# eduard-permyakov/permafrost-engine

Hardware: AMD Instinct MI355X
Metric: agent-steps/sec (+ flow-field cells/sec), every chunk field rebuilt + every agent stepped per tick (higher is better)
Workload: dtype u64-bitmask/u8 fields, f32 agents (f64 exp); 1 GPU; BASELINE configs[2]: 1024x1024 cells, 64 flow fields = 16384 chunk fields, 100000 agents; map_chunks=16, flow_fields=64, agents=100000, hz=20, dynamic_obstacles=0, parallelism=requests by destination + uid slabs x1, 1 all-gather (16 B/agent) per tick, ranks=1, rccl_ranks=1, backend=none, tile_exchange=auto, requests=reference planner fixture, has_dest_los=device lookup, initial_velocities=flow aligned, fields_ahead=True, tick_driver=c (navhip_tick_run), library=libnavhip.so (in-tree)

## Files before the change

permafrost-engine_amd/csrc/agent_internal.h:

```cpp
#pragma once
#define NH_SCAN_T 256
#include "navhip_internal.h"
#include "agent_types.h"

struct nh_spatial_scratch {
    int32_t *ent_cell, *ent_rank;
    int32_t *cell_count;
    int32_t *cell_start;
    int32_t *tmp_id;
    int32_t *block_sum;
    int32_t *box;
    int      box_parity;
    float4  *recA;
    float2  *recV;
    int32_t *pool_of;
    nh_pack_src src;
};

void nh_launch_spatial_build(nh_grid &G, const float *d_pos_xz, nh_spatial_scratch &S,
                             int slab_begin, int slab_end, hipStream_t s);
void nh_launch_agent_nbr(const nh_step_params &P, const nh_nbr &NB, hipStream_t s);
size_t nh_cohesion_scratch_bytes(int n_flocks, int n_members);
hipError_t nh_cohesion_scratch_reset(int32_t *scratch, int n_flocks, int n_members, hipStream_t s);
bool nh_launch_cohesion(const nh_step_params &P, int32_t *scratch, float *d_coh, int *parity, hipStream_t s);
void nh_launch_cohesion_regroup(const nh_step_params &P, int32_t *scratch, int *parity, hipStream_t s);
int nh_worklist_cap(int n_work);
bool nh_launch_agent_finish(const nh_step_params &P, const nh_nbr &NB, float *d_coh, nh_mid_rec *d_mid,
                            nh_worklists WL, int parity, const nh_step_outs &O, hipStream_t s,
                            hipStream_t side, navhip_ctx *ctx, bool *forked);
void nh_launch_state_update(const nh_step_params &P, const navhip_state_in &in, float4 *d_arrived, int32_t *d_arrived_n, uint8_t *d_state, uint8_t *d_flags,
                            hipStream_t s);
void nh_launch_region_lookup(const nh_step_params &P, int nq, const float *d_pos, const int32_t *d_rows,
                             const int32_t *d_centre_abs, const int32_t *d_radius, uint8_t *d_dir, uint8_t *d_at_slot,
                             hipStream_t s);
void nh_launch_spatial_query(const nh_grid &G, const float *d_query, int nq, float range, int maxout,
                             int32_t *d_counts, uint32_t *d_ids, hipStream_t s);
void nh_launch_clearpath(int nq, const float *ent, const float *des_v, const float *dyn,
                         const int32_t *n_dyn, const float *stat, const int32_t *n_stat, float *out,
                         int rows, hipStream_t s);
```

permafrost-engine_amd/csrc/agent_kernels.hip:

```cpp
#include "navhip_internal.h"
#include "agent_internal.h"
#include "agent_group.h"

__constant__ double c_exp2_64[64] = { NH_EXP2_64_TABLE };

#define SP_MAX_QUERY_R 30
__global__ __launch_bounds__(256) void k_sp_bbox(const float *pos_xz, int begin, int end, int32_t *box)
{
    __shared__ int32_t part[4][4];
    int32_t v[4] = {INT32_MIN, INT32_MIN, INT32_MIN, INT32_MIN};
    for(int i = begin + blockIdx.x * 256 + threadIdx.x; i < end; i += gridDim.x * 256) {
        const int32_t ix = bg_scale(pos_xz[2 * i]), iy = bg_scale(pos_xz[2 * i + 1]);
        v[0] = max(v[0], -ix); v[1] = max(v[1], ix); v[2] = max(v[2], -iy); v[3] = max(v[3], iy);
    }
#pragma unroll
    for(int q = 0; q < 4; q++) {
#pragma unroll
        for(int d = 32; d >= 1; d >>= 1) v[q] = max(v[q], __shfl_xor(v[q], d));
        if((threadIdx.x & 63) == 0) part[threadIdx.x >> 6][q] = v[q];
    }
    __syncthreads();
    if(threadIdx.x < 4) {
        int32_t m = INT32_MIN;
        for(int w = 0; w < 4; w++) m = max(m, part[w][threadIdx.x]);
// ... 900 lines not shown
    unit_totals(unit_end, 2 * NH_WL_SUB, [&](int k) { return (sub_cnt[k] + 3) >> 2; });
    __syncthreads();
    const int u = blockIdx.x * CPS_WAVES + wib;
    bool live = u < unit_end[2 * NH_WL_SUB - 1];
    int uid = 0;
    bool found = true;
    if(live) {
        const int k = first_above(unit_end, 2 * NH_WL_SUB, u), rel = u - (k ? unit_end[k - 1] : 0);
        const int list = NH_WL_ROW1 - k / NH_WL_SUB, sub = k % NH_WL_SUB;
        const int idx = rel * 4 + (lane >> 4);
        live = idx < sub_cnt[k];
        if(live) {
            uid = WL.ids[((size_t)list * NH_WL_SUB + sub) * WL.cap + idx];
            const nh_mid_rec R = mid[uid];
            const uint32_t c = NB.cnt[uid];
            const int n_dyn = (int)(c & 0xff), n_stat = (int)((c >> 8) & 0xff);
            cpent ent;
            ent.pos = mkv(P.pos_xz[2 * uid], P.pos_xz[2 * uid + 1]);
            ent.vel = mkv(P.vel_xz[2 * uid], P.vel_xz[2 * uid + 1]);
            ent.radius = P.radius[uid];
            const int gl = lane & 15;
            const bool have = gl < n_dyn + n_stat, isdyn = gl < n_dyn;
            cpent nb; nb.pos = mkv(0, 0); nb.vel = mkv(0, 0); nb.radius = 0;
            if(have) nb = nbr_load(NB, uid, isdyn ? gl : 32 + gl - n_dyn);
            const v2 nv = clearpath_small_row(ent, mkv(R.vpref[0], R.vpref[1]), nb, isdyn, have,
                                              cones[wib * 4 + (lane >> 4)], found);
            if(found && gl == 0)
                post_thread(P, uid, ent.pos, P.state[uid], P.flags[uid], ent.radius, nv, R.vel_cap, R.status, O);
        }
    }
    worklist_push(WL, NH_WL_RETRY, live && !found && (lane & 15) == 0, uid);
}

#define CP_ROWS_OCC 4
__attribute__((amdgpu_waves_per_eu(CP_ROWS_OCC, CP_ROWS_OCC)))
__global__ __launch_bounds__(CPR_WAVES * 64) void k_cp_rows(nh_step_params P, nh_nbr NB, const nh_mid_rec *mid,
                                                           nh_worklists WL, nh_step_outs O, int list0, int nlists,
                                                           int ticket_set, nh_signal lists_ready)
{
    if(lists_ready.flag && blockIdx.x == 0 && threadIdx.x == 0) {
#ifdef NH_HOSTSIM
        *lists_ready.flag = lists_ready.seq;
#else
        __hip_atomic_store(lists_ready.flag, lists_ready.seq, __ATOMIC_RELEASE, __HIP_MEMORY_SCOPE_AGENT);
#endif
    }
    __shared__ cp_lds<16> lds[CPR_WAVES * 4];
    __shared__ int32_t unit_end[4 * NH_WL_SUB];
    __shared__ int32_t sub_cnt[4 * NH_WL_SUB];
    asm volatile("" ::: "v127");
    static_assert(sizeof(cp_lds<16>) * CPR_WAVES * 4 + 8 * 4 * NH_WL_SUB >= sizeof(cp_lds<64>) * CP_WAVES + 8 * NH_WL_SUB + 4 + sizeof(cp_team),
                  "k_cp_rows' workgroup must own at least k_cp_heavy's LDS (hole inheritance)");
    const int wib = threadIdx.x >> 6, lane = threadIdx.x & 63;
    const int ntab = nlists * NH_WL_SUB;
    if(nlists == 1 && !__any(WL.count[list0 * NH_WL_SUB + lane] != 0)) return;
    for(int k = threadIdx.x; k < ntab; k += CPR_WAVES * 64)
        sub_cnt[k] = WL.count[(list0 - k / NH_WL_SUB) * NH_WL_SUB + k % NH_WL_SUB];
    __syncthreads();
    unit_totals(unit_end, ntab, [&](int k) { return (sub_cnt[k] + 3) >> 2; });
    __syncthreads();
    const int total = unit_end[ntab - 1];
    int32_t *counters = WL.count + NH_WL_LISTS * NH_WL_SUB + 32 * (1 + ticket_set * NH_CP_STRIPES);
    const int gw = blockIdx.x * CPR_WAVES + wib, nw = gridDim.x * CPR_WAVES;
    cp_lds<16> &S = lds[wib * 4 + (lane >> 4)];
    unit_draw D; D.round = 0;
    for(;;) {
        const int u = next_unit(D, counters, total, gw, nw, lane);
        if(u < 0) break;
        const int k = first_above(unit_end, ntab, u), rel = u - (k ? unit_end[k - 1] : 0);
        const int list = list0 - k / NH_WL_SUB, sub = k % NH_WL_SUB;
        const int idx = rel * 4 + (lane >> 4);
        if(idx < sub_cnt[k]) {
            const int uid = WL.ids[((size_t)list * NH_WL_SUB + sub) * WL.cap + idx];
            const nh_mid_rec R = mid[uid];
            const uint32_t c = NB.cnt[uid];
            const int n_dyn = (int)(c & 0xff), n_stat = (int)((c >> 8) & 0xff);
            cpent ent;
            ent.pos = mkv(P.pos_xz[2 * uid], P.pos_xz[2 * uid + 1]);
            ent.vel = mkv(P.vel_xz[2 * uid], P.vel_xz[2 * uid + 1]);
            ent.radius = P.radius[uid];
            cp_load_lists<16>(P.grid, NB, uid, n_dyn, n_stat, S);
            const v2 nv = clearpath_grp<16>(ent, mkv(R.vpref[0], R.vpref[1]), n_dyn, n_stat, S);
            if((lane & 15) == 0)
                post_thread(P, uid, ent.pos, P.state[uid], P.flags[uid], ent.radius, nv, R.vel_cap, R.status, O);
        }
    }
}

#define CP_HEAVY_OCC 4
__attribute__((amdgpu_waves_per_eu(CP_HEAVY_OCC, CP_HEAVY_OCC)))
__global__ __launch_bounds__(CP_WAVES * 64) void k_cp_heavy(nh_step_params P, nh_nbr NB, const nh_mid_rec *mid,
                                                            nh_worklists WL, nh_step_outs O, int32_t *zero_next)
{
    __shared__ cp_lds<64> lds[CP_WAVES];
    __shared__ int32_t hv_end[2 * NH_WL_SUB];
    __shared__ int32_t h_ticket;
    __shared__ cp_team team;
    const int wib = threadIdx.x >> 6, lane = threadIdx.x & 63;
    if(blockIdx.x == 0 && zero_next)
        for(int i = threadIdx.x; i < (int)NH_WL_COUNTERS; i += CP_WAVES * 64) zero_next[i] = 0;
    cp_lds<64> &S = lds[wib];
    if(!__any((WL.count[NH_WL_HEAVY * NH_WL_SUB + lane] | WL.count[NH_WL_WAVE * NH_WL_SUB + lane]) != 0)) return;
    unit_totals(hv_end, 2 * NH_WL_SUB, [&](int k) {
        return WL.count[(k < NH_WL_SUB ? NH_WL_HEAVY : NH_WL_WAVE) * NH_WL_SUB + k % NH_WL_SUB]; });
    __syncthreads();
    const int n_heavy = hv_end[2 * NH_WL_SUB - 1];
    int32_t *ticket = WL.count + NH_WL_LISTS * NH_WL_SUB;
    if(n_heavy >= CP_SOLO_MIN) {
        const int nw = (int)gridDim.x * CP_WAVES;
        for(int round = 0; ; round++) {
            int t = (int)blockIdx.x * CP_WAVES + wib;
            if(round > 0) {
                int v = 0x7fffffff;
                if(lane == 0 && nw + __atomic_load_n(ticket, __ATOMIC_RELAXED) < n_heavy) v = nw + atomicAdd(ticket, 1);
                t = __shfl(v, 0);
            }
            if(t >= n_heavy) break;
            const int k = first_above(hv_end, 2 * NH_WL_SUB, t), idx = t - (k ? hv_end[k - 1] : 0);
            const int uid = WL.ids[((size_t)(k < NH_WL_SUB ? NH_WL_HEAVY : NH_WL_WAVE) * NH_WL_SUB + k % NH_WL_SUB) * WL.cap + idx];
            const nh_mid_rec R = mid[uid];
            const uint32_t c = NB.cnt[uid];
            const int n_dyn = (int)(c & 0xff), n_stat = (int)((c >> 8) & 0xff);
            cpent ent;
            ent.pos = mkv(P.pos_xz[2 * uid], P.pos_xz[2 * uid + 1]);
            ent.vel = mkv(P.vel_xz[2 * uid], P.vel_xz[2 * uid + 1]);
            ent.radius = P.radius[uid];
            cp_load_lists<64>(P.grid, NB, uid, n_dyn, n_stat, S);
            const v2 nv = clearpath_grp<64>(ent, mkv(R.vpref[0], R.vpref[1]), n_dyn, n_stat, S);
            if(lane == 0)
                post_thread(P, uid, ent.pos, P.state[uid], P.flags[uid], ent.radius, nv, R.vel_cap, R.status, O);
        }
        return;
    }
    for(int round = 0; ; round++) {
        int t = blockIdx.x;
        if(round > 0) {
            __syncthreads();
            if(threadIdx.x == 0) {
                int v = 0x7fffffff;
                if((int)gridDim.x + __atomic_load_n(ticket, __ATOMIC_RELAXED) < n_heavy)
                    v = (int)gridDim.x + atomicAdd(ticket, 1);
                h_ticket = v;
            }
            __syncthreads();
            t = h_ticket;
        }
        if(t >= n_heavy) break;
        const int k = first_above(hv_end, 2 * NH_WL_SUB, t), idx = t - (k ? hv_end[k - 1] : 0);
        const int uid = WL.ids[((size_t)(k < NH_WL_SUB ? NH_WL_HEAVY : NH_WL_WAVE) * NH_WL_SUB + k % NH_WL_SUB) * WL.cap + idx];
        const nh_mid_rec R = mid[uid];
        const uint32_t c = NB.cnt[uid];
        const int n_dyn = (int)(c & 0xff), n_stat = (int)((c >> 8) & 0xff);
        cpent ent;
        ent.pos = mkv(P.pos_xz[2 * uid], P.pos_xz[2 * uid + 1]);
        ent.vel = mkv(P.vel_xz[2 * uid], P.vel_xz[2 * uid + 1]);
        ent.radius = P.radius[uid];
        const v2 vpref = mkv(R.vpref[0], R.vpref[1]);
        cp_load_lists<64>(P.grid, NB, uid, n_dyn, n_stat, S);
        const v2 nv = clearpath_grp<64, true>(ent, vpref, n_dyn, n_stat, S, wib, CP_WAVES, &team);
        if(wib == 0 && lane == 0)
            post_thread(P, uid, ent.pos, P.state[uid], P.flags[uid], ent.radius, nv, R.vel_cap, R.status, O);
    }
}

__global__ __launch_bounds__(AG_WAVES * 64) void k_agent_full(nh_step_params P, const float *coh_xz,
                                                              const nh_mid_rec *mid, nh_worklists WL,
                                                              nh_step_outs O, float scaled_max_force,
                                                              double force_thresh, int32_t *zero_next)
{
    __shared__ wave_lds lds[AG_WAVES];
    __shared__ cp_lds<64> cps[AG_WAVES];
    __shared__ double exp_tab[64];
    const int wib = threadIdx.x >> 6, lane = threadIdx.x & 63;
    if(blockIdx.x == 0 && zero_next)
        for(int i = threadIdx.x; i < (int)NH_WL_COUNTERS; i += AG_WAVES * 64) zero_next[i] = 0;
    if(!__any(WL.count[NH_WL_FULL * NH_WL_SUB + lane] != 0)) return;
    if(threadIdx.x < 64) exp_tab[threadIdx.x] = c_exp2_64[threadIdx.x];
    __syncthreads();
    wave_lds &W = lds[wib];
    cp_lds<64> &S = cps[wib];
    const nh_grid &G = P.grid;
    for(int sub = 0; sub < NH_WL_SUB; sub++) {
    const int count = WL.count[NH_WL_FULL * NH_WL_SUB + sub];
    for(int idx = blockIdx.x * AG_WAVES + wib; idx < count; idx += gridDim.x * AG_WAVES) {
        const int uid = WL.ids[((size_t)NH_WL_FULL * NH_WL_SUB + sub) * WL.cap + idx];
        const nh_mid_rec R = mid[uid];
        const uint32_t my_slot = (uint32_t)G.pool_of[uid];
        const uint32_t my_bits = slot_bits(G, my_slot);
        const v2 me = mkv(P.pos_xz[2 * uid], P.pos_xz[2 * uid + 1]);
        const v2 vel = mkv(P.vel_xz[2 * uid], P.vel_xz[2 * uid + 1]);
        const float my_radius = P.radius[uid];
        int n30raw = -1;
        v2 vpref = mkv(0.0f, 0.0f);
        wave_sync();
        if(R.mode != AM_ZERO_VPREF) {
            int n30 = sp_query_wave(G, me.x, me.z, 30.0f, 128, W.ids30, lane, W.d2_30);
            wave_sync();
            n30raw = n30;
            const int n10d = derive_r10(G, me, W.ids30, W.d2_30, n30raw, W.ids10d, lane);
            n30 = filter_garrisoned_wave(G, W.ids30, n30, lane);
            if(n10d < 0) n30raw = -1; else n30raw = n10d;
            const v2 separation = separation_wave(G, my_slot, me, my_radius, my_bits, W.ids30, n30,
                                                  W.u.sep, scaled_max_force, lane, exp_tab);
            vpref = vpref_from_forces(P, uid, R.mode, me, vel, P.flock[uid], mkv(R.arrive[0], R.arrive[1]),
                                      separation, R.probes, coh_xz, scaled_max_force, force_thresh);
        }
        uint32_t *ids10 = W.u.ids10;
        int n10;
        if(n30raw >= 0) {
            ids10 = W.ids10d;
            n10 = n30raw;
        }else{
            n10 = sp_query_wave(G, me.x, me.z, 10.0f, 512, W.u.ids10, lane);
            wave_sync();
        }
        n10 = filter_garrisoned_wave(G, ids10, n10, lane);
        int n_dyn, n_stat;
        classify_neighbours(G, my_slot, my_bits, ids10, n10, S.dyn, n_dyn, S.stat, n_stat, lane);
        cpent ent; ent.pos = me; ent.vel = vel; ent.radius = my_radius;
        const v2 nv = clearpath_grp<64>(ent, vpref, n_dyn, n_stat, S);
        if(lane == 0) {
            if(O.vpref_xz) { O.vpref_xz[2 * uid] = vpref.x; O.vpref_xz[2 * uid + 1] = vpref.z; }
            post_thread(P, uid, me, P.state[uid], P.flags[uid], my_radius, nv, R.vel_cap, R.status, O);
        }
    }
    }
}

__global__ __launch_bounds__(256) void k_spatial_query(nh_grid G, const float *query_xz, int nq,
                                                       float range, int maxout, int32_t *out_counts,
                                                       uint32_t *out_ids)
{
    const int q = (blockIdx.x * 256 + threadIdx.x) >> 6, lane = threadIdx.x & 63;
    if(q >= nq) return;
    uint32_t *mine = out_ids + (size_t)q * maxout;
    int n = sp_query_wave(G, query_xz[2 * q], query_xz[2 * q + 1], range, maxout, mine, lane);
    wave_sync();
    for(int k = lane; k < n; k += 64) mine[k] = slot_bits(G, mine[k]) >> NH_PB_UID_SHIFT;
    if(lane == 0) out_counts[q] = n;
}

__global__ __launch_bounds__(256) void k_arrived_compact(nh_step_params P, float4 *arrived, int32_t *arrived_n)
{
    __shared__ int count;
    const int f = blockIdx.x;
    if(threadIdx.x == 0) count = 0;
    __syncthreads();
    const int b = P.flock_offsets[f], e = P.flock_offsets[f + 1];
    for(int k0 = b; k0 < e; k0 += 256) {
        const int k = k0 + (int)threadIdx.x;
        int m = -1;
        if(k < e) { m = P.flock_members[k]; if(P.state[m] != NAVHIP_STATE_ARRIVED) m = -1; }
        const uint64_t bal = __ballot(m >= 0);
        int base = 0;
        if((threadIdx.x & 63) == 0 && bal) base = atomicAdd(&count, __popcll(bal));
        base = __shfl(base, 0);
        if(m >= 0) {
            const int at = b + base + __popcll(bal & ((1ull << (threadIdx.x & 63)) - 1ull));
            if(at < P.n_ents) arrived[at] = make_float4(P.pos_xz[2 * m], P.pos_xz[2 * m + 1], P.radius[m], __int_as_float(m));
// ... 298 lines not shown
{
    if(!(P.n_ents > 0 && P.n_flocks > 0 && P.n_members > 0)) return false;
    const coh_scratch C = coh_layout(scratch, P.n_flocks, P.n_members);
    const int nwaves = (P.n_members + 15) / 16 + P.n_flocks;
    const int prev = *parity ^ 1;
    if(P.n_flocks <= COH_INLINE_PLAN_MAX) {
        hipLaunchKernelGGL(k_cohesion<true>, dim3(nwaves), dim3(64), 0, s, P, (const int32_t*)C.wave_off,
                           (const int32_t*)C.perm[prev], (const int32_t*)C.valid, d_coh, (const int32_t*)C.bin_start,
                           (const int32_t*)C.saved[prev]);
        return true;
    }
    hipLaunchKernelGGL(k_coh_plan, dim3(1), dim3(256), 0, s, (const int32_t*)C.bin_start, P.flock_offsets,
                       (const int32_t*)C.saved[prev], P.n_flocks, P.work_begin, P.work_end, P.members_key, C.wave_off, C.valid);
    hipLaunchKernelGGL(k_cohesion<false>, dim3(nwaves), dim3(64), 0, s, P, (const int32_t*)C.wave_off,
                       (const int32_t*)C.perm[prev], (const int32_t*)C.valid, d_coh, (const int32_t*)C.bin_start,
                       (const int32_t*)C.saved[prev]);
    return true;
}

void nh_launch_cohesion_regroup(const nh_step_params &P, int32_t *scratch, int *parity, hipStream_t s)
{
    const coh_scratch C = coh_layout(scratch, P.n_flocks, P.n_members);
    coh_regroup(P, C, *parity, s);
    *parity ^= 1;
}
int nh_worklist_cap(int n_work)
{
    const int waves = (n_work + 63) / 64;
    return ((waves + NH_WL_SUB - 1) / NH_WL_SUB) * 64 + 16;
}

bool nh_launch_agent_finish(const nh_step_params &P, const nh_nbr &NB, float *d_coh, nh_mid_rec *d_mid,
                            nh_worklists WL, int parity, const nh_step_outs &O, hipStream_t s,
                            hipStream_t side, navhip_ctx *ctx, bool *forked)
{
    const int nwork = P.work_end - P.work_begin;
    if(!(P.n_ents > 0 && nwork > 0)) return false;
    const float smf = (float)((double)(0.75f / (float)P.hz) * 20.0);
    const double thresh = ((double)(0.75f / (float)P.hz) * 20.0) * 0.01;
    int32_t *zero_next = WL.count + (parity ^ 1) * NH_WL_COUNTERS;
    WL.count += parity * NH_WL_COUNTERS;
    hipLaunchKernelGGL(k_agent_mid, dim3((nwork + 63) / 64), dim3(64), 0, s, P, NB, (const float*)d_coh, d_mid, WL, O, smf, thresh);
    const bool fork = side != nullptr && side != s;
    hipStream_t sh = fork ? side : s;
    const nh_signal lists_ready = fork ? nh_handover_by_kernel(ctx, NH_HO_MID, s) : nh_signal{nullptr, 0};
    *forked = fork;
    const int nblk = min(4096 / CP_WAVES, (nwork + 15) / 16 + 1);
    const int nblk_rows = min(4096 / CPR_WAVES, (nwork + 15) / 16 * (CP_WAVES / CPR_WAVES) + 1);
    hipLaunchKernelGGL(k_cp_rows, dim3(nblk_rows), dim3(CPR_WAVES * 64), 0, s, P, NB, (const nh_mid_rec*)d_mid, WL, O,
                       (int)NH_WL_ROW3, 2, 0, lists_ready);
    if(fork) nh_handover_wait(ctx, NH_HO_MID, sh);
    hipLaunchKernelGGL(k_cp_small, dim3((nwork / 4 + 2 * NH_WL_SUB + CPS_WAVES - 1) / CPS_WAVES + 1), dim3(CPS_WAVES * 64), 0, sh, P, NB,
                       (const nh_mid_rec*)d_mid, WL, O);
    hipLaunchKernelGGL(k_cp_rows, dim3(64 * CP_WAVES / CPR_WAVES), dim3(CPR_WAVES * 64), 0, sh, P, NB, (const nh_mid_rec*)d_mid, WL, O,
                       (int)NH_WL_RETRY, 1, 1, nh_signal{nullptr, 0});
    hipLaunchKernelGGL(k_cp_heavy, dim3(nblk), dim3(CP_WAVES * 64), 0, sh, P, NB, (const nh_mid_rec*)d_mid, WL, O, zero_next);
    if(fork) nh_handover_signal(ctx, NH_HO_CP, sh);
    hipLaunchKernelGGL(k_agent_full, dim3(min(1024, (nwork + AG_WAVES - 1) / AG_WAVES)), dim3(AG_WAVES * 64), 0, s, P,
                       (const float*)d_coh, (const nh_mid_rec*)d_mid, WL, O, smf, thresh, (int32_t*)nullptr);
    if(fork) nh_handover_wait(ctx, NH_HO_CP, s, -1, NH_HO_END);
    return true;
}

void nh_launch_spatial_query(const nh_grid &G, const float *d_query, int nq, float range, int maxout,
                             int32_t *d_counts, uint32_t *d_ids, hipStream_t s)
{
    if(nq > 0)
        hipLaunchKernelGGL(k_spatial_query, dim3((nq + 3) / 4), dim3(256), 0, s, G, d_query, nq, range,
                           maxout, d_counts, d_ids);
}

void nh_launch_clearpath(int nq, const float *ent, const float *des_v, const float *dyn,
                         const int32_t *n_dyn, const float *stat, const int32_t *n_stat, float *out,
                         int rows, hipStream_t s)
{
    if(nq <= 0) return;
    if(rows == 2)
        hipLaunchKernelGGL(k_clearpath_team, dim3(nq), dim3(CP_WAVES * 64), 0, s, nq, ent, des_v, dyn,
                           n_dyn, stat, n_stat, out);
    else if(rows)
        hipLaunchKernelGGL(k_clearpath<16>, dim3((nq + 7) / 8), dim3(128), 0, s, nq, ent, des_v, dyn,
                           n_dyn, stat, n_stat, out);
    else
        hipLaunchKernelGGL(k_clearpath<64>, dim3((nq + 1) / 2), dim3(128), 0, s, nq, ent, des_v, dyn,
                           n_dyn, stat, n_stat, out);
}
```

permafrost-engine_amd/csrc/agent_types.h:

```cpp
#pragma once
#include <stdint.h>
#include <stddef.h>
#include "map_view.h"

#ifdef NH_HOSTSIM
struct float2 { float x, y; };
struct float4 { float x, y, z, w; };
static inline float2 make_float2(float x, float y) { float2 r = {x, y}; return r; }
static inline float4 make_float4(float x, float y, float z, float w) { float4 r = {x, y, z, w}; return r; }
#endif

#define NH_PB_MOVABLE     0x01u
#define NH_PB_AIR         0x02u
#define NH_PB_GARRISONED  0x04u
#define NH_PB_STATIC      0x08u
#define NH_PB_WATER       0x10u
#define NH_PB_IDLE        0x20u
#define NH_PB_UID_SHIFT   8

struct nh_grid {
    int32_t origin_x, origin_y;
    int     grid_w, grid_h;
    int     n;
    const int32_t *cell_start;
// ... 36 lines not shown
    const float    *los_pos_xz;
    const int32_t  *region_row;
    const int32_t  *region_field_slot;
};

struct nh_step_outs {
    float   *vel_xz, *new_pos_xz, *vdes_xz, *vpref_xz;
    uint8_t *status;
};

#define NH_NB_IRREGULAR 0x1u
#define NH_NB_DONE      0x2u
struct nh_nbr {
    float2   *sep;
    uint32_t *cnt;
    float    *rec;
    int       stride;
};

enum { NH_WL_ROW0 = 0, NH_WL_ROW1, NH_WL_ROW2, NH_WL_ROW3,
       NH_WL_WAVE,
       NH_WL_HEAVY,
       NH_WL_FULL,
       NH_WL_RETRY,
       NH_WL_LISTS };
#define NH_WL_SUB 64
struct nh_worklists {
    int32_t *count;
    int32_t *ids;
    int      cap;
};
#define NH_CP_STRIPES 32
#define NH_WL_COUNTERS (NH_WL_LISTS * NH_WL_SUB + 32 * (2 + 2 * NH_CP_STRIPES))

struct nh_mid_rec {
    float    vpref[2];
    float    vdes[2];
    float    arrive[2];
    uint16_t probes;
    uint8_t  status;
    uint8_t  mode;
    float    vel_cap;
};
```

permafrost-engine_amd/csrc/navhip_internal.h:

```cpp
#pragma once
#include <hip/hip_runtime.h>
#include <stdint.h>
#include <string>
#include <vector>
#include <initializer_list>
#include <stddef.h>
#include "navhip.h"
#include "map_view.h"

static_assert(sizeof(navhip_field_req) == 32, "navhip_field_req must stay 32 bytes");
static_assert(sizeof(navhip_los_req) == 16, "navhip_los_req must stay 16 bytes");

#define NH_CELLS   4096
#define NH_RES     64
#define NH_INF_U32 0x3fffffffu

#define HIPCHK(ctx, expr)                                                                   \
    do {                                                                                    \
        hipError_t _e = (expr);                                                             \
        if(_e != hipSuccess) {                                                              \
            (ctx)->last_error = std::string(#expr) + ": " + hipGetErrorString(_e);          \
            return NAVHIP_ERR_DEVICE;                                                       \
        }                                                                                   \
    } while(0)
// ... 200 lines not shown
{
    nh_buf *one[] = {&ctx->d_reqs, &ctx->d_dirs, &ctx->d_integ, &ctx->d_dirty_list, &ctx->gen_list, &ctx->state_arrived,
                     &ctx->state_arrived_n};
    for(nh_buf *b : one) f(*b);
    for(auto &b : ctx->step.buf) f(b);
    for(auto &b : ctx->stage) f(b);
}

enum { NH_STREAM_SIDE0 = 0,
       NH_STREAM_SIDE1,
       NH_STREAM_MAIN,
       NH_STREAM_FIELDS,
       NH_STREAM_COMM,
       NH_STREAM_FIXED };
int         nh_streams_for(navhip_ctx *ctx, hipStream_t main, hipStream_t out[NH_STREAM_FIXED]);
hipStream_t nh_stream_partial_for(navhip_ctx *ctx, hipStream_t main, int cu_begin, int cu_count);
bool        nh_streams_alive(int device);
void        nh_streams_forget(int device, hipStream_t s);
int         nh_ensure_side_streams(navhip_ctx *ctx, hipStream_t main);

struct nh_signal { int32_t *flag; int32_t seq; };
struct nh_handover {
    int32_t *flags;
    int32_t *status;
    int32_t *status_dev;
    int32_t  seq[NH_HO_FLAGS];
    bool       forced_events, never_events, by_events;
    hipEvent_t ev[NH_HO_FLAGS];
};
void     nh_handover_mode(navhip_ctx *ctx, bool jam);
int      nh_handover_ensure(navhip_ctx *ctx);
void     nh_handover_destroy(navhip_ctx *ctx);
nh_signal nh_handover_by_kernel(navhip_ctx *ctx, int flag, hipStream_t producer);
void     nh_handover_signal(navhip_ctx *ctx, int flag, hipStream_t producer);
void     nh_handover_wait(navhip_ctx *ctx, int flag, hipStream_t consumer, int before = -1, int after = -1);
void     nh_handover_wait2(navhip_ctx *ctx, int flag_a, int flag_b, hipStream_t consumer);
int32_t  nh_handover_seq(navhip_ctx *ctx, int flag);
void     nh_handover_wait_for(navhip_ctx *ctx, int flag, int32_t want, hipStream_t consumer);
bool     nh_handover_failed(navhip_ctx *ctx);

extern "C" int nh_validate_field_reqs(navhip_ctx *ctx, const navhip_field_req *reqs, int n);
int  navhip_build_fields_slots_dev(navhip_ctx *ctx, const navhip_field_req *dev_reqs, int n, uint8_t *dev_fields,
                                   const int32_t *dev_slots, hipStream_t s);
int  nh_ensure(navhip_ctx *ctx, nh_buf &b, size_t need);
int  nh_ensure_buf(navhip_ctx *ctx, nh_buf &b, size_t need);
int  nh_stage_in(navhip_ctx *ctx, nh_stage_slot slot, const void *host, size_t bytes, const void **dst, hipStream_t s);
int  nh_stage_world(navhip_ctx *ctx, const navhip_world *w, navhip_world *d, hipStream_t s, std::initializer_list<size_t> only = {});
int  nh_stage_reserve(navhip_ctx *ctx, nh_stage_slot slot, size_t bytes, void **dev);
void nh_async_destroy(navhip_ctx *ctx);
void nh_async_invalidate_static(navhip_ctx *ctx);
bool nh_async_resident(navhip_ctx *ctx, navhip_world *w, navhip_step_out *o);
int  nh_async_slabs(navhip_ctx *ctx, size_t in_bytes, size_t out_bytes, char **h_in, char **h_out);
bool nh_is_pinned(const void *p);
int  nh_refresh_derived(navhip_ctx *ctx, hipStream_t s);
int  nh_spatial_query_dev(navhip_ctx *ctx, const navhip_world *dev_w, const float *d_query, int nq, float range, int maxout,
                          int32_t *d_counts, uint32_t *d_ids, hipStream_t s);
const uint8_t *nh_pool_fields(const navhip_ctx *ctx);
const int32_t *nh_pool_map(const navhip_ctx *ctx);
int nh_pool_dests(const navhip_ctx *ctx);
int nh_pool_slots(const navhip_ctx *ctx);

void nh_launch_derive(navhip_ctx *ctx, int layer, const uint32_t *d_chunk_list, int n,
                      hipStream_t s);
int  nh_launch_fields(navhip_ctx *ctx, const navhip_field_req *d_reqs, int n, uint8_t *d_dirs,
                      float *d_integ, int32_t *d_gen_list, hipStream_t s,
                      const int32_t *d_out_slot = nullptr);

void nh_launch_blockers_circles(navhip_ctx *ctx, const navhip_circle *d_circles, int n, float map_x,
                                float map_z, hipStream_t s);
// ... 8 lines not shown
```

permafrost-engine_amd/csrc/step_api.hip:

```cpp
#include "navhip_internal.h"
#include "agent_internal.h"
#include "agent_thread.h"
#include <cmath>

#include <algorithm>
#include <cstring>
#include <initializer_list>

enum sb_fresh : uint8_t {
    SB_ANYTHING,
    SB_ZEROED,
    SB_EMPTY_BOXES,
};
struct sb_need { nh_step_buf buf; size_t bytes; sb_fresh fresh; };

template<size_t N> static int step_bufs_ensure(navhip_ctx *ctx, const sb_need (&needs)[N], hipStream_t s)
{
    for(const sb_need &n : needs) {
        nh_buf &b = ctx->step.buf[n.buf];
        const void *old = b.p;
        int rc = nh_ensure_buf(ctx, b, n.bytes);
        if(rc) return rc;
        if(b.p == old) continue;
        if(n.fresh == SB_ZEROED) HIPCHK(ctx, hipMemsetAsync(b.p, 0, b.cap, s));
// ... 306 lines not shown
        HIPCHK(ctx, hipEventRecord(ctx->step.ev_regroup, ctx->step.aux[1]));
        ctx->step.regroup_pending = true;
    }
    HIPCHK(ctx, hipGetLastError());
    ctx->step.pre.valid = true;
    ctx->step.pre.key = prefetch_key(w, P);
    return NAVHIP_OK;
}

int navhip_agent_prefetch_dev(navhip_ctx *ctx, const navhip_world *w, void *stream)
{
    return navhip_agent_prefetch_dev_ex(ctx, w, stream, 0);
}

static int send_step_lists(navhip_ctx *ctx, int parity_used, hipStream_t fallback, bool on_fallback)
{
    if(!ctx->step.lists_pinned) {
        HIPCHK(ctx, hipHostMalloc((void**)&ctx->step.lists_pinned, sizeof(int32_t) * NH_WL_LISTS * NH_WL_SUB, hipHostMallocDefault));
        memset(ctx->step.lists_pinned, 0, sizeof(int32_t) * NH_WL_LISTS * NH_WL_SUB);
    }
    const int32_t *src = step_buf<const int32_t>(ctx, NH_SB_WL_COUNT) + parity_used * NH_WL_COUNTERS;
    HIPCHK(ctx, hipMemcpyAsync(ctx->step.lists_pinned, src, sizeof(int32_t) * NH_WL_LISTS * NH_WL_SUB, hipMemcpyDeviceToHost,
                               (ctx->step.aux[0] && !on_fallback) ? ctx->step.aux[0] : fallback));
    return NAVHIP_OK;
}

static int step_tail(navhip_ctx *ctx, const nh_step_params &P, const nh_nbr &NB, const nh_worklists &WL, const nh_step_outs &O,
                     hipStream_t s)
{
    nh_step_state &st = ctx->step;
    const bool serial = st.serial_step;
    bool forked = false;
    if(nh_launch_agent_finish(P, NB, step_buf<float>(ctx, NH_SB_COH), step_buf<nh_mid_rec>(ctx, NH_SB_MIDREC), WL, st.wl_parity, O, s,
                              serial ? nullptr : st.aux[0], ctx, &forked)) {
        st.lists_signalled = forked;
        if(forked) {
            st.step_end_on = ctx->ho->by_events ? nullptr : s;
            st.step_end_signalled = true;
        }
        int rc = send_step_lists(ctx, st.wl_parity, s, serial);
        st.wl_parity ^= 1;
        if(rc) return rc;
    }
    HIPCHK(ctx, hipGetLastError());
    return NAVHIP_OK;
}

int navhip_agent_step_dev(navhip_ctx *ctx, const navhip_world *w, const navhip_step_out *out,
                          void *stream)
{
    if(!ctx || !out || !out->vel_xz) return NAVHIP_ERR_INVALID;
    int rc = step_check_world(ctx, w);
    if(rc) return rc;
    if(w->n_ents == 0) return NAVHIP_OK;
    if(nh_handover_failed(ctx)) return NAVHIP_ERR_DEVICE;
    HIPCHK(ctx, hipSetDevice(ctx->device));
    hipStream_t s = stream ? (hipStream_t)stream : ctx->stream;
    ctx->step.step_end_on = nullptr; ctx->step.step_end_signalled = false;

    nh_step_params P;
    rc = step_fill_params(ctx, w, &P);
    if(rc) return rc;
    if(!grid_geometry(w, &P.grid)) {
        ctx->last_error = "agent step: empty spatial-grid bounds";
        return NAVHIP_ERR_INVALID;
    }
    ctx->counters.step_calls++; ctx->counters.agent_steps += (uint64_t)(P.work_end - P.work_begin);
// ... 195 lines not shown
```

permafrost-engine_amd/csrc/stream_set.hip:

```cpp
#include "navhip_internal.h"
#include <array>
#include <chrono>
#include <cstdio>
#include <cstdlib>
#include <cstring>
#include <map>
#include <mutex>
#include <utility>
#include <vector>

#define NH_PIPES 4
__global__ void k_nh_spin(long long ticks, int32_t *word, int32_t seq)
{
#ifndef NH_HOSTSIM
    const long long t0 = wall_clock64();
    while(wall_clock64() - t0 < ticks) { }
    if(word) __hip_atomic_store(word, seq, __ATOMIC_RELEASE, __HIP_MEMORY_SCOPE_AGENT);
#else
    if(word) *word = seq;
#endif
}

__global__ void k_ho_signal(int32_t *flag, int32_t seq)
{
#ifdef NH_HOSTSIM
    *flag = seq;
#else
    __hip_atomic_store(flag, seq, __ATOMIC_RELEASE, __HIP_MEMORY_SCOPE_AGENT);
#endif
}
__global__ void k_ho_wait(const int32_t *flag, int32_t want, int32_t *status, nh_signal before, nh_signal after)
{
#ifdef NH_HOSTSIM
    if(before.flag) *before.flag = before.seq;
    if(*flag - want < 0) { fprintf(stderr, "k_ho_wait: the producer of a hand-over was enqueued behind its consumer\n"); abort(); }
    if(after.flag) *after.flag = after.seq;
#else
    if(before.flag) __hip_atomic_store(before.flag, before.seq, __ATOMIC_RELEASE, __HIP_MEMORY_SCOPE_AGENT);
    const long long t0 = wall_clock64();
    while(__hip_atomic_load(flag, __ATOMIC_RELAXED, __HIP_MEMORY_SCOPE_AGENT) - want < 0) {
        __builtin_amdgcn_s_sleep(8);
        if(wall_clock64() - t0 > 200000000LL) {
            __hip_atomic_store(status, 1, __ATOMIC_RELAXED, __HIP_MEMORY_SCOPE_SYSTEM);
            break;
        }
    }
    __atomic_thread_fence(__ATOMIC_ACQUIRE);
    if(after.flag) __hip_atomic_store(after.flag, after.seq, __ATOMIC_RELEASE, __HIP_MEMORY_SCOPE_AGENT);
#endif
}

__global__ void k_ho_wait2(const int32_t *flag_a, int32_t want_a, const int32_t *flag_b, int32_t want_b, int32_t *status)
{
#ifdef NH_HOSTSIM
    if(*flag_a - want_a < 0 || *flag_b - want_b < 0) { fprintf(stderr, "k_ho_wait2: the producer of a hand-over was enqueued behind its consumer\n"); abort(); }
#else
    const long long t0 = wall_clock64();
    while(__hip_atomic_load(flag_a, __ATOMIC_RELAXED, __HIP_MEMORY_SCOPE_AGENT) - want_a < 0 ||
          __hip_atomic_load(flag_b, __ATOMIC_RELAXED, __HIP_MEMORY_SCOPE_AGENT) - want_b < 0) {
        __builtin_amdgcn_s_sleep(8);
        if(wall_clock64() - t0 > 200000000LL) {
            __hip_atomic_store(status, 1, __ATOMIC_RELAXED, __HIP_MEMORY_SCOPE_SYSTEM);
            break;
        }
    }
    __atomic_thread_fence(__ATOMIC_ACQUIRE);
#endif
}

int nh_handover_ensure(navhip_ctx *ctx)
{
    if(ctx->ho) return NAVHIP_OK;
    nh_handover *H = new nh_handover();
    memset(H, 0, sizeof(*H));
    if(hipMalloc((void**)&H->flags, sizeof(int32_t) * NH_HO_FLAGS * NH_HO_STRIDE) != hipSuccess ||
       hipMemset(H->flags, 0, sizeof(int32_t) * NH_HO_FLAGS * NH_HO_STRIDE) != hipSuccess ||
       hipHostMalloc((void**)&H->status, sizeof(int32_t), hipHostMallocMapped) != hipSuccess ||
       hipHostGetDevicePointer((void**)&H->status_dev, H->status, 0) != hipSuccess) {
        (void)hipGetLastError();
        if(H->flags) hipFree(H->flags);
        if(H->status) hipHostFree(H->status);
        delete H;
        ctx->last_error = "hand-over words: out of memory";
        return NAVHIP_ERR_NOMEM;
    }
    *H->status = 0;
    const char *mode = getenv("NAVHIP_HANDOVER"), *pmc = getenv("ROCPROF_COUNTER_COLLECTION");
    const bool serialised = pmc && *pmc && strcmp(pmc, "0") && strcmp(pmc, "False") && strcmp(pmc, "false");
    H->forced_events = H->by_events = mode ? !strcmp(mode, "events") : serialised;
    H->never_events = mode && !strcmp(mode, "words");
    if(!H->never_events)
        for(auto &e : H->ev)
            if(hipEventCreateWithFlags(&e, hipEventDisableTiming) != hipSuccess) { ctx->last_error = "hand-over events"; ctx->ho = H; nh_handover_destroy(ctx); return NAVHIP_ERR_DEVICE; }
    ctx->ho = H;
    return NAVHIP_OK;
}

void nh_handover_destroy(navhip_ctx *ctx)
{
    if(!ctx->ho) return;
    for(auto &e : ctx->ho->ev) if(e) hipEventDestroy(e);
    hipFree(ctx->ho->flags);
    hipHostFree(ctx->ho->status);
    delete ctx->ho;
    ctx->ho = nullptr;
}

void nh_handover_mode(navhip_ctx *ctx, bool jam)
{
    nh_handover *H = ctx->ho;
    H->by_events = H->forced_events || (jam && !H->never_events);
}

nh_signal nh_handover_by_kernel(navhip_ctx *ctx, int flag, hipStream_t producer)
{
    nh_handover *H = ctx->ho;
    ++H->seq[flag];
    if(H->by_events) { hipEventRecord(H->ev[flag], producer); return nh_signal{nullptr, 0}; }
    return nh_signal{H->flags + flag * NH_HO_STRIDE, H->seq[flag]};
}

void nh_handover_signal(navhip_ctx *ctx, int flag, hipStream_t producer)
{
    nh_handover *H = ctx->ho;
    if(H->by_events) { ++H->seq[flag]; hipEventRecord(H->ev[flag], producer); return; }
    hipLaunchKernelGGL(k_ho_signal, dim3(1), dim3(1), 0, producer, H->flags + flag * NH_HO_STRIDE, ++H->seq[flag]);
}

void nh_handover_wait(navhip_ctx *ctx, int flag, hipStream_t consumer, int before, int after)
{
    nh_handover *H = ctx->ho;
    if(H->by_events) {
        if(before >= 0) { ++H->seq[before]; hipEventRecord(H->ev[before], consumer); }
        hipStreamWaitEvent(consumer, H->ev[flag], 0);
        if(after >= 0) { ++H->seq[after]; hipEventRecord(H->ev[after], consumer); }
        return;
    }
    const int32_t want = H->seq[flag];
    nh_signal b = {nullptr, 0}, a = {nullptr, 0};
    if(before >= 0) { b.flag = H->flags + before * NH_HO_STRIDE; b.seq = ++H->seq[before]; }
    if(after >= 0)  { a.flag = H->flags + after * NH_HO_STRIDE;  a.seq = ++H->seq[after]; }
    hipLaunchKernelGGL(k_ho_wait, dim3(1), dim3(1), 0, consumer, (const int32_t*)(H->flags + flag * NH_HO_STRIDE), want,
                       H->status_dev, b, a);
}

void nh_handover_wait_for(navhip_ctx *ctx, int flag, int32_t want, hipStream_t consumer)
{
    nh_handover *H = ctx->ho;
    if(H->by_events) { hipStreamWaitEvent(consumer, H->ev[flag], 0); return; }
    hipLaunchKernelGGL(k_ho_wait, dim3(1), dim3(1), 0, consumer, (const int32_t*)(H->flags + flag * NH_HO_STRIDE), want,
                       H->status_dev, nh_signal{nullptr, 0}, nh_signal{nullptr, 0});
}

int32_t nh_handover_seq(navhip_ctx *ctx, int flag) { return ctx->ho->seq[flag]; }

void nh_handover_wait2(navhip_ctx *ctx, int flag_a, int flag_b, hipStream_t consumer)
{
    nh_handover *H = ctx->ho;
    if(H->by_events) { hipStreamWaitEvent(consumer, H->ev[flag_a], 0); hipStreamWaitEvent(consumer, H->ev[flag_b], 0); return; }
    hipLaunchKernelGGL(k_ho_wait2, dim3(1), dim3(1), 0, consumer, (const int32_t*)(H->flags + flag_a * NH_HO_STRIDE), H->seq[flag_a],
                       (const int32_t*)(H->flags + flag_b * NH_HO_STRIDE), H->seq[flag_b], H->status_dev);
}

bool nh_handover_failed(navhip_ctx *ctx)
{
    if(!ctx->ho || !*(volatile int32_t*)ctx->ho->status) return false;
    ctx->last_error = "a hand-over between two streams of the agent step was not signalled within two seconds (under a profiler "
                      "that serialises kernels -- rocprofv3 --pmc -- run with NAVHIP_HANDOVER=events)";
    return true;
}

namespace {
struct nh_dev_streams {
    bool        ready = false;
    hipStream_t full[NH_PIPES] = {};
    std::map<std::pair<int, int>, std::array<hipStream_t, NH_PIPES>> partial;
    std::map<hipStream_t, int> caller_pipe;
    int32_t    *words = nullptr, *status = nullptr, *status_dev = nullptr;
    int32_t     seq = 0;
    bool        unmeasured = false;
    double      base_us = 0.0;
    int         measured_pairs = 0, collisions_seen = 0;
};
#define NH_SAME_PIPE 1.6
std::mutex g_streams_mu;
std::map<int, nh_dev_streams> g_streams;

hipStream_t masked_stream(navhip_ctx *ctx, int cu_begin, int cu_count)
{
    hipDeviceProp_t prop;
    if(hipGetDeviceProperties(&prop, ctx->device) != hipSuccess) { ctx->last_error = "hipGetDeviceProperties failed"; return nullptr; }
    const int ncu = prop.multiProcessorCount;
    if(cu_count <= 0 || cu_begin + cu_count > ncu) cu_count = ncu - cu_begin;
    uint32_t mask[32] = {0};
// ... 172 lines not shown
```

Before: 39.22 million agent-steps/s.

## Run agent_full on a second side stream and signal completion from last workgroup

Moves k_agent_full off the main stream onto a second auxiliary stream, so it runs alongside the heavy clearpath chain. Both kernels now signal completion from their last finishing workgroup through an atomic counter and a release store, replacing a separate one-thread signal kernel launch. The main stream then waits on both flags with one two-flag wait kernel. This removes a launch and serialisation point per tick, at the cost of extra atomics, cross-stream spin-waits and more handover-protocol complexity.

Result: slower. 38.43 million agent-steps/s (-2.0%).

```diff
diff --git a/permafrost-engine_amd/csrc/agent_internal.h b/permafrost-engine_amd/csrc/agent_internal.h
--- a/permafrost-engine_amd/csrc/agent_internal.h
+++ b/permafrost-engine_amd/csrc/agent_internal.h
@@ -27,7 +27,7 @@
 int nh_worklist_cap(int n_work);
 bool nh_launch_agent_finish(const nh_step_params &P, const nh_nbr &NB, float *d_coh, nh_mid_rec *d_mid,
                             nh_worklists WL, int parity, const nh_step_outs &O, hipStream_t s,
-                            hipStream_t side, navhip_ctx *ctx, bool *forked);
+                            hipStream_t side, hipStream_t side1, navhip_ctx *ctx, bool *forked);
 void nh_launch_state_update(const nh_step_params &P, const navhip_state_in &in, float4 *d_arrived, int32_t *d_arrived_n, uint8_t *d_state, uint8_t *d_flags,
                             hipStream_t s);
 void nh_launch_region_lookup(const nh_step_params &P, int nq, const float *d_pos, const int32_t *d_rows,
diff --git a/permafrost-engine_amd/csrc/agent_kernels.hip b/permafrost-engine_amd/csrc/agent_kernels.hip
--- a/permafrost-engine_amd/csrc/agent_kernels.hip
+++ b/permafrost-engine_amd/csrc/agent_kernels.hip
@@ -956,6 +956,19 @@
     worklist_push(WL, NH_WL_RETRY, live && !found && (lane & 15) == 0, uid);
 }
 
+__device__ __forceinline__ void last_workgroup_stores(int32_t *counter, nh_signal done)
+{
+    if(!done.flag) return;
+#ifdef NH_HOSTSIM
+    if(threadIdx.x == 0 && atomicAdd(counter, 1) == (int)gridDim.x - 1) *done.flag = done.seq;
+#else
+    __threadfence();
+    __syncthreads();
+    if(threadIdx.x == 0 && __hip_atomic_fetch_add(counter, 1, __ATOMIC_ACQ_REL, __HIP_MEMORY_SCOPE_AGENT) == (int)gridDim.x - 1)
+        __hip_atomic_store(done.flag, done.seq, __ATOMIC_RELEASE, __HIP_MEMORY_SCOPE_AGENT);
+#endif
+}
+
 #define CP_ROWS_OCC 4
 __attribute__((amdgpu_waves_per_eu(CP_ROWS_OCC, CP_ROWS_OCC)))
 __global__ __launch_bounds__(CPR_WAVES * 64) void k_cp_rows(nh_step_params P, nh_nbr NB, const nh_mid_rec *mid,
@@ -1011,20 +1024,11 @@
     }
 }
 
-#define CP_HEAVY_OCC 4
-__attribute__((amdgpu_waves_per_eu(CP_HEAVY_OCC, CP_HEAVY_OCC)))
-__global__ __launch_bounds__(CP_WAVES * 64) void k_cp_heavy(nh_step_params P, nh_nbr NB, const nh_mid_rec *mid,
-                                                            nh_worklists WL, nh_step_outs O, int32_t *zero_next)
-{
-    __shared__ cp_lds<64> lds[CP_WAVES];
-    __shared__ int32_t hv_end[2 * NH_WL_SUB];
-    __shared__ int32_t h_ticket;
-    __shared__ cp_team team;
+__device__ __forceinline__ void cp_heavy_drain(const nh_step_params &P, const nh_nbr &NB, const nh_mid_rec *mid, const nh_worklists &WL,
+                                               const nh_step_outs &O, cp_lds<64> *lds, int32_t *hv_end, int32_t &h_ticket, cp_team &team)
+{
     const int wib = threadIdx.x >> 6, lane = threadIdx.x & 63;
-    if(blockIdx.x == 0 && zero_next)
-        for(int i = threadIdx.x; i < (int)NH_WL_COUNTERS; i += CP_WAVES * 64) zero_next[i] = 0;
     cp_lds<64> &S = lds[wib];
-    if(!__any((WL.count[NH_WL_HEAVY * NH_WL_SUB + lane] | WL.count[NH_WL_WAVE * NH_WL_SUB + lane]) != 0)) return;
     unit_totals(hv_end, 2 * NH_WL_SUB, [&](int k) {
         return WL.count[(k < NH_WL_SUB ? NH_WL_HEAVY : NH_WL_WAVE) * NH_WL_SUB + k % NH_WL_SUB]; });
     __syncthreads();
@@ -1087,18 +1091,33 @@
     }
 }
 
+#define CP_HEAVY_OCC 4
+__attribute__((amdgpu_waves_per_eu(CP_HEAVY_OCC, CP_HEAVY_OCC)))
+__global__ __launch_bounds__(CP_WAVES * 64) void k_cp_heavy(nh_step_params P, nh_nbr NB, const nh_mid_rec *mid,
+                                                            nh_worklists WL, nh_step_outs O, int32_t *zero_next, nh_signal done)
+{
+    __shared__ cp_lds<64> lds[CP_WAVES];
+    __shared__ int32_t hv_end[2 * NH_WL_SUB];
+    __shared__ int32_t h_ticket;
+    __shared__ cp_team team;
+    const int lane = threadIdx.x & 63;
+    if(blockIdx.x == 0 && zero_next)
+        for(int i = threadIdx.x; i < (int)NH_WL_COUNTERS; i += CP_WAVES * 64) zero_next[i] = 0;
+    if(__any((WL.count[NH_WL_HEAVY * NH_WL_SUB + lane] | WL.count[NH_WL_WAVE * NH_WL_SUB + lane]) != 0))
+        cp_heavy_drain(P, NB, mid, WL, O, lds, hv_end, h_ticket, team);
+    last_workgroup_stores(WL.count + NH_WL_DONE, done);
+}
+
 __global__ __launch_bounds__(AG_WAVES * 64) void k_agent_full(nh_step_params P, const float *coh_xz,
                                                               const nh_mid_rec *mid, nh_worklists WL,
                                                               nh_step_outs O, float scaled_max_force,
-                                                              double force_thresh, int32_t *zero_next)
+                                                              double force_thresh, nh_signal done)
 {
     __shared__ wave_lds lds[AG_WAVES];
     __shared__ cp_lds<64> cps[AG_WAVES];
     __shared__ double exp_tab[64];
     const int wib = threadIdx.x >> 6, lane = threadIdx.x & 63;
-    if(blockIdx.x == 0 && zero_next)
-        for(int i = threadIdx.x; i < (int)NH_WL_COUNTERS; i += AG_WAVES * 64) zero_next[i] = 0;
-    if(!__any(WL.count[NH_WL_FULL * NH_WL_SUB + lane] != 0)) return;
+    if(__any(WL.count[NH_WL_FULL * NH_WL_SUB + lane] != 0)) {
     if(threadIdx.x < 64) exp_tab[threadIdx.x] = c_exp2_64[threadIdx.x];
     __syncthreads();
     wave_lds &W = lds[wib];
@@ -1149,6 +1168,8 @@
         }
     }
     }
+    }
+    last_workgroup_stores(WL.count + NH_WL_DONE + 1, done);
 }
 
 __global__ __launch_bounds__(256) void k_spatial_query(nh_grid G, const float *query_xz, int nq,
@@ -1513,7 +1534,7 @@
 
 bool nh_launch_agent_finish(const nh_step_params &P, const nh_nbr &NB, float *d_coh, nh_mid_rec *d_mid,
                             nh_worklists WL, int parity, const nh_step_outs &O, hipStream_t s,
-                            hipStream_t side, navhip_ctx *ctx, bool *forked)
+                            hipStream_t side, hipStream_t side1, navhip_ctx *ctx, bool *forked)
 {
     const int nwork = P.work_end - P.work_begin;
     if(!(P.n_ents > 0 && nwork > 0)) return false;
@@ -1523,7 +1544,7 @@
     WL.count += parity * NH_WL_COUNTERS;
     hipLaunchKernelGGL(k_agent_mid, dim3((nwork + 63) / 64), dim3(64), 0, s, P, NB, (const float*)d_coh, d_mid, WL, O, smf, thresh);
     const bool fork = side != nullptr && side != s;
-    hipStream_t sh = fork ? side : s;
+    hipStream_t sh = fork ? side : s, sf = fork && side1 ? side1 : s;
     const nh_signal lists_ready = fork ? nh_handover_by_kernel(ctx, NH_HO_MID, s) : nh_signal{nullptr, 0};
     *forked = fork;
     const int nblk = min(4096 / CP_WAVES, (nwork + 15) / 16 + 1);
@@ -1535,11 +1556,18 @@
                        (const nh_mid_rec*)d_mid, WL, O);
     hipLaunchKernelGGL(k_cp_rows, dim3(64 * CP_WAVES / CPR_WAVES), dim3(CPR_WAVES * 64), 0, sh, P, NB, (const nh_mid_rec*)d_mid, WL, O,
                        (int)NH_WL_RETRY, 1, 1, nh_signal{nullptr, 0});
-    hipLaunchKernelGGL(k_cp_heavy, dim3(nblk), dim3(CP_WAVES * 64), 0, sh, P, NB, (const nh_mid_rec*)d_mid, WL, O, zero_next);
-    if(fork) nh_handover_signal(ctx, NH_HO_CP, sh);
-    hipLaunchKernelGGL(k_agent_full, dim3(min(1024, (nwork + AG_WAVES - 1) / AG_WAVES)), dim3(AG_WAVES * 64), 0, s, P,
-                       (const float*)d_coh, (const nh_mid_rec*)d_mid, WL, O, smf, thresh, (int32_t*)nullptr);
-    if(fork) nh_handover_wait(ctx, NH_HO_CP, s, -1, NH_HO_END);
+    const nh_signal chain_done = fork ? nh_handover_by_kernel_end(ctx, NH_HO_CP) : nh_signal{nullptr, 0};
+    hipLaunchKernelGGL(k_cp_heavy, dim3(nblk), dim3(CP_WAVES * 64), 0, sh, P, NB, (const nh_mid_rec*)d_mid, WL, O, zero_next, chain_done);
+    if(fork) nh_handover_kernel_ended(ctx, NH_HO_CP, sh);
+    const nh_signal full_done = sf != s ? nh_handover_by_kernel_end(ctx, NH_HO_COH) : nh_signal{nullptr, 0};
+    if(sf != s) nh_handover_wait(ctx, NH_HO_MID, sf);
+    hipLaunchKernelGGL(k_agent_full, dim3(min(1024, (nwork + AG_WAVES - 1) / AG_WAVES)), dim3(AG_WAVES * 64), 0, sf, P,
+                       (const float*)d_coh, (const nh_mid_rec*)d_mid, WL, O, smf, thresh, full_done);
+    if(sf != s) nh_handover_kernel_ended(ctx, NH_HO_COH, sf);
+    if(fork) {
+        if(sf != s) nh_handover_wait2(ctx, NH_HO_CP, NH_HO_COH, s, NH_HO_END);
+        else        nh_handover_wait(ctx, NH_HO_CP, s, -1, NH_HO_END);
+    }
     return true;
 }
 
diff --git a/permafrost-engine_amd/csrc/agent_types.h b/permafrost-engine_amd/csrc/agent_types.h
--- a/permafrost-engine_amd/csrc/agent_types.h
+++ b/permafrost-engine_amd/csrc/agent_types.h
@@ -92,6 +92,7 @@
 };
 #define NH_CP_STRIPES 32
 #define NH_WL_COUNTERS (NH_WL_LISTS * NH_WL_SUB + 32 * (2 + 2 * NH_CP_STRIPES))
+#define NH_WL_DONE     (NH_WL_LISTS * NH_WL_SUB + 32 * (1 + 2 * NH_CP_STRIPES))
 
 struct nh_mid_rec {
     float    vpref[2];
diff --git a/permafrost-engine_amd/csrc/navhip_internal.h b/permafrost-engine_amd/csrc/navhip_internal.h
--- a/permafrost-engine_amd/csrc/navhip_internal.h
+++ b/permafrost-engine_amd/csrc/navhip_internal.h
@@ -256,9 +256,11 @@
 int      nh_handover_ensure(navhip_ctx *ctx);
 void     nh_handover_destroy(navhip_ctx *ctx);
 nh_signal nh_handover_by_kernel(navhip_ctx *ctx, int flag, hipStream_t producer);
+nh_signal nh_handover_by_kernel_end(navhip_ctx *ctx, int flag);
+void     nh_handover_kernel_ended(navhip_ctx *ctx, int flag, hipStream_t producer);
 void     nh_handover_signal(navhip_ctx *ctx, int flag, hipStream_t producer);
 void     nh_handover_wait(navhip_ctx *ctx, int flag, hipStream_t consumer, int before = -1, int after = -1);
-void     nh_handover_wait2(navhip_ctx *ctx, int flag_a, int flag_b, hipStream_t consumer);
+void     nh_handover_wait2(navhip_ctx *ctx, int flag_a, int flag_b, hipStream_t consumer, int after = -1);
 int32_t  nh_handover_seq(navhip_ctx *ctx, int flag);
 void     nh_handover_wait_for(navhip_ctx *ctx, int flag, int32_t want, hipStream_t consumer);
 bool     nh_handover_failed(navhip_ctx *ctx);
diff --git a/permafrost-engine_amd/csrc/step_api.hip b/permafrost-engine_amd/csrc/step_api.hip
--- a/permafrost-engine_amd/csrc/step_api.hip
+++ b/permafrost-engine_amd/csrc/step_api.hip
@@ -362,7 +362,7 @@
     const bool serial = st.serial_step;
     bool forked = false;
     if(nh_launch_agent_finish(P, NB, step_buf<float>(ctx, NH_SB_COH), step_buf<nh_mid_rec>(ctx, NH_SB_MIDREC), WL, st.wl_parity, O, s,
-                              serial ? nullptr : st.aux[0], ctx, &forked)) {
+                              serial ? nullptr : st.aux[0], serial ? nullptr : st.aux[1], ctx, &forked)) {
         st.lists_signalled = forked;
         if(forked) {
             st.step_end_on = ctx->ho->by_events ? nullptr : s;
diff --git a/permafrost-engine_amd/csrc/stream_set.hip b/permafrost-engine_amd/csrc/stream_set.hip
--- a/permafrost-engine_amd/csrc/stream_set.hip
+++ b/permafrost-engine_amd/csrc/stream_set.hip
@@ -50,10 +50,11 @@
 #endif
 }
 
-__global__ void k_ho_wait2(const int32_t *flag_a, int32_t want_a, const int32_t *flag_b, int32_t want_b, int32_t *status)
+__global__ void k_ho_wait2(const int32_t *flag_a, int32_t want_a, const int32_t *flag_b, int32_t want_b, int32_t *status, nh_signal after)
 {
 #ifdef NH_HOSTSIM
     if(*flag_a - want_a < 0 || *flag_b - want_b < 0) { fprintf(stderr, "k_ho_wait2: the producer of a hand-over was enqueued behind its consumer\n"); abort(); }
+    if(after.flag) *after.flag = after.seq;
 #else
     const long long t0 = wall_clock64();
     while(__hip_atomic_load(flag_a, __ATOMIC_RELAXED, __HIP_MEMORY_SCOPE_AGENT) - want_a < 0 ||
@@ -65,6 +66,7 @@
         }
     }
     __atomic_thread_fence(__ATOMIC_ACQUIRE);
+    if(after.flag) __hip_atomic_store(after.flag, after.seq, __ATOMIC_RELEASE, __HIP_MEMORY_SCOPE_AGENT);
 #endif
 }
 
@@ -120,6 +122,18 @@
     return nh_signal{H->flags + flag * NH_HO_STRIDE, H->seq[flag]};
 }
 
+nh_signal nh_handover_by_kernel_end(navhip_ctx *ctx, int flag)
+{
+    nh_handover *H = ctx->ho;
+    ++H->seq[flag];
+    return H->by_events ? nh_signal{nullptr, 0} : nh_signal{H->flags + flag * NH_HO_STRIDE, H->seq[flag]};
+}
+
+void nh_handover_kernel_ended(navhip_ctx *ctx, int flag, hipStream_t producer)
+{
+    if(ctx->ho->by_events) hipEventRecord(ctx->ho->ev[flag], producer);
+}
+
 void nh_handover_signal(navhip_ctx *ctx, int flag, hipStream_t producer)
 {
     nh_handover *H = ctx->ho;
@@ -154,12 +168,18 @@
 
 int32_t nh_handover_seq(navhip_ctx *ctx, int flag) { return ctx->ho->seq[flag]; }
 
-void nh_handover_wait2(navhip_ctx *ctx, int flag_a, int flag_b, hipStream_t consumer)
-{
-    nh_handover *H = ctx->ho;
-    if(H->by_events) { hipStreamWaitEvent(consumer, H->ev[flag_a], 0); hipStreamWaitEvent(consumer, H->ev[flag_b], 0); return; }
+void nh_handover_wait2(navhip_ctx *ctx, int flag_a, int flag_b, hipStream_t consumer, int after)
+{
+    nh_handover *H = ctx->ho;
+    if(H->by_events) {
+        hipStreamWaitEvent(consumer, H->ev[flag_a], 0); hipStreamWaitEvent(consumer, H->ev[flag_b], 0);
+        if(after >= 0) { ++H->seq[after]; hipEventRecord(H->ev[after], consumer); }
+        return;
+    }
+    nh_signal a = {nullptr, 0};
+    if(after >= 0) { a.flag = H->flags + after * NH_HO_STRIDE; a.seq = ++H->seq[after]; }
     hipLaunchKernelGGL(k_ho_wait2, dim3(1), dim3(1), 0, consumer, (const int32_t*)(H->flags + flag_a * NH_HO_STRIDE), H->seq[flag_a],
-                       (const int32_t*)(H->flags + flag_b * NH_HO_STRIDE), H->seq[flag_b], H->status_dev);
+                       (const int32_t*)(H->flags + flag_b * NH_HO_STRIDE), H->seq[flag_b], H->status_dev, a);
 }
 
 bool nh_handover_failed(navhip_ctx *ctx)
```
